# loqalabs/loqa-hub

Measured on AMD Instinct MI355X. Metric: utterances_per_sec (multi-command utterances; ms per added command reported alongside), higher is better.
Workload: dtype bf16

## Files before the change

### csrc/kernels/gemm_ws.hip

```cpp
#include "gemm_mfma.h"

struct GemmWsParams {
  const void* x; long long ldx;
  const void* w;
  int M, N, K;
  int epi, act;
  const float* bias;
  void* y; long long ldy;
  int bm;
  int S;
  float* ws;
  int* counters;
};

template <int FM, int NBW, int NBX, int EPI>
__global__ __launch_bounds__(512) void gemm_ws_kernel(GemmWsParams p) {
  constexpr int WN = 2, WM = 4, NW = 8, FN = 4;
  constexpr int TN = 16 * FN, TM = 16 * FM;
  constexpr int BN = TN * WN, BM = TM * WM;
  constexpr int WSTAGE = BN * 128, XSTAGE = BM * 128;
  constexpr int IW = BN / 8 / NW;
  constexpr int IX = BM / 8 / NW;
  static_assert(IW * 8 * NW == BN && IX * 8 * NW == BM, "stage rows split evenly over the waves");
  static_assert(NBW >= 2 && NBX >= 2 && NBX <= NBW, "stage depths");
  __shared__ __attribute__((aligned(1024))) unsigned char lds[NBW * WSTAGE + NBX * XSTAGE];
  unsigned char* const wl = lds;
  unsigned char* const xl = lds + NBW * WSTAGE;

  const int lane = threadIdx.x & 63;
  const int wave = __builtin_amdgcn_readfirstlane(threadIdx.x >> 6);
  const int wn = wave % WN, wm = wave / WN;
  const int M = p.M, N = p.N;
  const int mblocks = (M + p.bm - 1) / p.bm;
  const int tiles = mblocks * (N / BN), S = p.S;
  const int id = xcd_remap(blockIdx.x, gridDim.x);
  const int s = id / tiles, tile = id - s * tiles;
  const int mb = tile % mblocks, nb = tile / mblocks;
  const int m0 = mb * p.bm, n0 = nb * BN;
  const int KT = p.K / GEMM_BK;
  const int kt0 = (int)(((long long)s * KT) / S), kt1 = (int)(((long long)(s + 1) * KT) / S);
  const int nt = kt1 - kt0;
  const bf16_t* __restrict__ X = reinterpret_cast<const bf16_t*>(p.x);
  const bf16_t* __restrict__ W = reinterpret_cast<const bf16_t*>(p.w);

  const bf16_t* wsrc[IW];
#pragma unroll
  for (int i = 0; i < IW; ++i) {
    const int r = stage_row(wave * IW + i, lane), c = stage_chunk(r, lane);
    wsrc[i] = W + (size_t)weight_row<EPI == EPI_SWIGLU, TN>(r, n0, N) * p.K + (size_t)kt0 * GEMM_BK + c * 8;
  }
  const bf16_t* xsrc[IX];
#pragma unroll
  for (int i = 0; i < IX; ++i) {
    const int r = stage_row(wave * IX + i, lane), c = stage_chunk(r, lane);
    const int m = min(m0 + min(r, p.bm - 1), M - 1);
    xsrc[i] = X + (size_t)m * p.ldx + (size_t)kt0 * GEMM_BK + c * 8;
  }
  auto stage_w = [&](int kt) { stage_issue<IW>(wsrc, kt * GEMM_BK, wl + (kt % NBW) * WSTAGE, wave); };
  auto stage_x = [&](int kt) { stage_issue<IX>(xsrc, kt * GEMM_BK, xl + (kt % NBX) * XSTAGE, wave); };

  float4v acc[FN][FM];
  acc_zero(acc);
  const int fr = lane & 15, fq = lane >> 4;

  static_assert(NBW == 3 && (NBX == 2 || NBX == 3), "the counted waits below assume these depths");
  for (int v = -(NBW - 1); v < 0; ++v) {
    if (v + NBX - 1 >= 0 && v + NBX - 1 < nt) stage_x(v + NBX - 1);
    if (v + NBW - 1 < nt) stage_w(v + NBW - 1);
  }
  for (int t = 0; t < nt; ++t) {
    if (t + 1 < nt) {
      if constexpr (NBX == 2) wait_vm<IW>();
      else wait_vm<IW + IX>();
    } else {
      wait_vm<0>();
    }
    __builtin_amdgcn_s_barrier();
    if (t + NBX - 1 < nt) stage_x(t + NBX - 1);
    if (t + NBW - 1 < nt) stage_w(t + NBW - 1);
    mfma_step(wl + (t % NBW) * WSTAGE, wn * TN, xl + (t % NBX) * XSTAGE, wm * TM, fr, fq, acc);
  }

  if (S > 1 && !splitk_reduce<FN, FM, NW>(p.ws, p.counters, tile, s, S, reinterpret_cast<int*>(lds), wave, lane, acc))
    return;
  epi_store<EPI>(acc, EpiOut{p.y, p.ldy, p.bias, p.act, nullptr, 0}, m0 + wm * TM, min(M, m0 + p.bm),
                 n0 + wn * TN, N, 0, fr, fq);
}

template <int FM, int NBW, int NBX>
static int ws_launch(const GemmWsParams& p, hipStream_t st) {
  const int grid = ((p.M + p.bm - 1) / p.bm) * (p.N / 128) * p.S;
  switch (p.epi) {
    case EPI_SWIGLU:
      hipLaunchKernelGGL((gemm_ws_kernel<FM, NBW, NBX, EPI_SWIGLU>), dim3(grid), dim3(512), 0, st, p);
      break;
    case EPI_RESID:
      hipLaunchKernelGGL((gemm_ws_kernel<FM, NBW, NBX, EPI_RESID>), dim3(grid), dim3(512), 0, st, p);
      break;
    default:
      hipLaunchKernelGGL((gemm_ws_kernel<FM, NBW, NBX, EPI_BF16>), dim3(grid), dim3(512), 0, st, p);
  }
  return (int)hipGetLastError();
}

extern "C" int loqa_gemm_ws(const GemmWsParams* p, int depth, hipStream_t st) {
  if (!p || p->M <= 0 || p->epi < 0 || p->epi > EPI_RESID || !p->x || !p->w || !p->y)
    return (int)hipErrorInvalidValue;
  if (p->N % 128 || p->K % GEMM_BK || p->K < GEMM_BK || p->ldx % 8 || p->ldy % 4 || p->bm < 64 || p->bm % 64 ||
      p->bm > 384 || depth < 0 || depth > 1 || p->S < 1 || p->S > p->K / GEMM_BK)
    return (int)hipErrorInvalidValue;
  if (p->S > 1 && (!p->ws || !p->counters)) return (int)hipErrorInvalidValue;
  if ((p->epi == EPI_SWIGLU && (p->bias || p->act)) || (p->epi == EPI_RESID && p->act))
    return (int)hipErrorInvalidValue;
  const int fm = p->bm / 64;
  if (depth == 1) {
    switch (fm) {
      case 1: return ws_launch<1, 3, 3>(*p, st);
      case 2: return ws_launch<2, 3, 3>(*p, st);
      case 3: return ws_launch<3, 3, 3>(*p, st);
      case 4: return ws_launch<4, 3, 3>(*p, st);
      default: return (int)hipErrorInvalidValue;
    }
  }
  switch (fm) {
    case 1: return ws_launch<1, 3, 2>(*p, st);
    case 2: return ws_launch<2, 3, 2>(*p, st);
    case 3: return ws_launch<3, 3, 2>(*p, st);
    case 4: return ws_launch<4, 3, 2>(*p, st);
    case 5: return ws_launch<5, 3, 2>(*p, st);
    case 6: return ws_launch<6, 3, 2>(*p, st);
    default: return (int)hipErrorInvalidValue;
  }
}
```

### loqa_hub_amd/ops/__init__.py

```python
from __future__ import annotations

import copy
import ctypes
import math
import os

import torch

from . import reference as ref
from . import _lib
from ._lib import FusedParams, check, kernels, ptr, stream_ptr


def _gpu(t: torch.Tensor) -> bool:
    return t.is_cuda


def _bf16_contig(t: torch.Tensor, name: str) -> None:
    if t.dtype != torch.bfloat16:
        raise TypeError(f"{name} must be bfloat16, got {t.dtype}")
    if not t.is_contiguous():
        raise ValueError(f"{name} must be contiguous")


# ... 1441 lines not shown

    def __init__(self, w: torch.Tensor, *, norm: str | None = None, norm_w=None, norm_b=None,
                 bias=None, perm: torch.Tensor | None = None):
        wf = w.float()
        self.norm = norm
        if norm is not None:
            wf = wf * norm_w.float()[None, :]
        wb = wf.to(torch.bfloat16)
        b = torch.zeros(w.shape[0], dtype=torch.float32, device=w.device)
        if bias is not None:
            b = b + bias.float()
        if norm == "ln" and norm_b is not None:
            b = b + (w.float() * norm_b.float()[None, :]).sum(1)
        self.colsum = wb.float().sum(1) if norm == "ln" else None
        self.has_bias = bias is not None or (norm == "ln" and norm_b is not None)
        if perm is not None:
            wb = wb[perm]
            b = b[perm]
            if self.colsum is not None:
                self.colsum = self.colsum[perm].contiguous()
        self.bias = b.contiguous() if self.has_bias else None
        self.wp = shuffle_weight(wb.contiguous())
        self.N, self.K = w.shape


def tune_fused(wp, mode: str, *, mpads=(16, 32, 64, 128), norm=None, act: str = "none",
               heads: tuple | None = None, cos_sin=None, prefill: bool = False,
               xl: bool = True) -> None:
    lin = wp if isinstance(wp, FusedLinear) else None
    w = lin.wp if lin is not None else wp
    if not _gpu(w) or NO_TUNE:
        return
    dev = w.device
    N, K = w.shape[0] * 16, w.shape[1] * 32
    scr = FusedScratch(dev)
    bf = dict(dtype=torch.bfloat16, device=dev)
    nrm = norm if norm is not None else (lin.norm if lin is not None else None)
    nbytes = w.numel() * w.element_size()
    copies = [wp]
    for _ in range(min(15, -(-(768 << 20) // nbytes) - 1)):
        if lin is not None:
            c = copy.copy(lin)
            c.wp = lin.wp.clone()
        else:
            c = wp.clone()
        copies.append(c)
    xl_on = xl and os.environ.get("LOQA_TUNE_XL", "1") != "0"
    for Mpad in mpads:
        if Mpad == 128 and not xl_on:
            continue
        key = (mode, N, K, Mpad) + _wtag(w)
        if key in _FSPLITS:
            continue
        x = torch.randn(Mpad, K, **bf)
        kw: dict = {}
        if nrm:
            tiles = max(1, K // 32)
            scr.rowsq[: tiles * Mpad].fill_(float(K) / tiles)
            kw.update(rowsq_tiles=tiles)
        if mode == "resid":
            kw.update(residual=torch.zeros(Mpad, N, **bf))
        elif mode == "act":
            kw.update(act=act)
        elif mode == "rope":
            H, Hkv, D = heads
            kc = torch.zeros(max(4, Mpad // 16), Hkv, 16, D, **bf)
            pos = torch.arange(Mpad, dtype=torch.int32, device=dev)
            kw.update(positions=pos, cos_sin=cos_sin, q_out=torch.empty(Mpad, H * D, **bf),
                      k_cache=kc, v_cache=torch.zeros_like(kc), slots=pos, n_heads=H, n_kv=Hkv,
                      head_dim=D)
        wide = Mpad <= 32 or prefill
        rts = (1, 2, 4) if (prefill and Mpad == 64) else (1, 2)
        xl = "only" if Mpad == 128 else "no"
        tune_fused_splits(key, lambda sp, rt, wr, i, xl_=0: skinny_fused(
            x, copies[i], mode, scr, splits=sp, rt=rt, wr=wr, norm=nrm, xl=xl_, **kw), K, rts=rts,
            ncopies=len(copies), wr4=wide, fewest=wide, xl=xl)
    del copies


def fold_norm(w: torch.Tensor, norm_w: torch.Tensor) -> torch.Tensor:
    return (w.float() * norm_w.float()[None, :]).to(w.dtype)


def skinny_fused(x: torch.Tensor, wp, mode: str, scratch: FusedScratch, *,
                 splits: int | None = None, norm=None, eps: float = 1e-5,
                 rowsq_tiles: int | None = None, rt: int | None = None,
                 residual: torch.Tensor | None = None, positions=None, cos_sin=None, q_out=None,
                 k_cache=None, v_cache=None, slots=None, n_heads: int = 0, n_kv: int = 0,
                 head_dim: int = 0, out=None, act: str = "none", bias=None, colsum=None,
                 row_sums: bool = False, wr: int | None = None, xl: int | None = None,
                 attn: dict | None = None) -> torch.Tensor:
    if attn is not None:
        assert mode in ("rope", "act")
        rope = mode == "rope"
        if not rope and out is None:
            out = torch.empty(x.shape[0], wp.shape[0] * 16 if not isinstance(wp, FusedLinear)
                              else wp.N, dtype=torch.bfloat16, device=x.device)
        qq = skinny_fused(x, wp, mode, scratch, splits=splits, norm=norm, eps=eps,
                          rowsq_tiles=rowsq_tiles, rt=rt, positions=positions, cos_sin=cos_sin,
                          q_out=q_out, k_cache=k_cache, v_cache=v_cache, slots=slots,
                          n_heads=n_heads, n_kv=n_kv, head_dim=head_dim, bias=bias,
                          colsum=colsum, wr=wr, xl=xl, out=out, act=act)
        if rope:
            return attention(q_out, k_cache, v_cache, attn["cu_q"], n_heads=n_heads,
                             n_kv=n_kv, head_dim=head_dim, causal=True, max_q=attn["max_q"],
                             ctx_lens=attn["ctx_lens"], block_tables=attn["block_tables"],
                             scale=attn.get("scale"), grouped=True,
                             split_keys=attn["split_keys"], num_splits=attn["num_splits"],
                             workspace=attn["workspace"], out=attn.get("out"),
                             max_k=attn.get("max_k"))
        return attention(qq, attn["k"], attn["v"], attn["cu_q"], n_heads=n_heads, n_kv=n_kv,
                         head_dim=head_dim, causal=False, max_q=attn["max_q"],
                         cu_k=attn["kv_start"], ctx_lens=attn["ctx_lens"],
                         scale=attn.get("scale"), grouped=True,
                         split_keys=attn["split_keys"], num_splits=attn["num_splits"],
                         workspace=attn["workspace"], out=attn.get("out"))
    if isinstance(wp, FusedLinear):
        lin = wp
        wp = lin.wp
        norm = lin.norm if norm is None else norm
        bias = lin.bias if bias is None else bias
        colsum = lin.colsum if colsum is None else colsum
    Mpad, K = x.shape
    N = wp.shape[0] * 16
    nrm = _NORMS[norm]
    fp8, mx4 = isinstance(wp, Fp8Weight), isinstance(wp, Mxfp4Weight)
    tuned = _FSPLITS.get((mode, N, K, Mpad) + _wtag(wp))
    S = splits or (tuned[0] if tuned else choose_splits(N, K, Mpad, tag=_wtag(wp)))
    rt = rt or (tuned[1] if tuned else (1 if Mpad == 128 else 2))
    if xl is None:
        xl = tuned[3] if (tuned and not splits and len(tuned) > 3) else int(Mpad == 128)
    if wr is None:
        wr = tuned[2] if (tuned and not splits and len(tuned) > 2) else 1
        if mx4 and wr == 1 and not xl and K % (S * 512):
            S, wr = 1, 4
            rt = rt if N % (64 * rt) == 0 else 1
    if xl:
        wr = 4
        rt = rt if rt in (1, 2) and N % (64 * rt) == 0 else 1
    elif wr != 1 and (S != 1 or N % (64 * rt)):
        wr = 1
    if rowsq_tiles is None:
        rowsq_tiles = scratch.stat_tiles
    m = _FUSED_MODES[mode]
    ntiles = N // (16 * rt)
    if mode == "resid":
        scratch.stat_tiles = ntiles
    if mode == "silu" and out is None:
        out = torch.empty(Mpad, N // 2, dtype=torch.bfloat16, device=x.device)
    elif mode == "act" and out is None:
        out = torch.empty(Mpad, N, dtype=torch.float32 if act == "f32" else torch.bfloat16,
                          device=x.device)
    if not _gpu(x):
        return _skinny_fused_ref(x, wp, mode, scratch, nrm, eps, rowsq_tiles, residual,
                                 positions, cos_sin, q_out, k_cache, v_cache, slots, n_heads,
                                 n_kv, head_dim, out, act, bias, colsum, row_sums, rt)
    assert Mpad in (16, 32, 64, 128) and x.dtype == torch.bfloat16 and x.stride(1) == 1
    assert Mpad != 128 or xl, "Mpad 128 needs the XL layout"
    assert ntiles <= scratch.counters.numel() and ntiles * Mpad <= scratch.rowsq.numel()
    if nrm == 2:
        assert colsum is not None and colsum.numel() == N
    if fp8:
        assert nrm != 2, "fp8 weights: no LayerNorm prologue"
        assert wp.is_cuda and wp.wp.is_contiguous() and wp.scale.is_contiguous()
    elif mx4:
        assert nrm != 2, "MXFP4 weights: no LayerNorm prologue"
        assert wp.is_cuda and wp.wp.is_contiguous() and wp.scales.is_contiguous()
        assert wp.wp.data_ptr() % 16 == 0 and wp.scales.data_ptr() % 4 == 0
    else:
        _bf16_contig(wp, "wp")
    if bias is not None:
        assert bias.dtype == torch.float32 and bias.numel() == N and bias.is_contiguous()
    if mode == "act":
        assert out.dtype == (torch.float32 if act == "f32" else torch.bfloat16)
        assert out.stride(0) % 4 == 0 and out.shape[0] >= Mpad and out.shape[1] >= N
    if mode == "rope":
        assert slots.numel() >= Mpad and q_out.shape[0] >= Mpad and k_cache.is_contiguous()
        assert cos_sin is None or positions.numel() >= Mpad
    elif mode == "resid":
        assert residual.shape[0] >= Mpad and residual.shape[1] == N
    part = torch.empty(S, Mpad, N, dtype=torch.float32, device=x.device) if S > 1 else None
    blk = k_cache.shape[2] if k_cache is not None else 0
    p = FusedParams()
    p.x, p.ldx, p.Wp, p.part, p.counters = ptr(x), x.stride(0), ptr(wp.wp if fp8 or mx4 else wp), \
        ptr(part), ptr(scratch.counters)
    if fp8:
        p.wdtype, p.wscale = 1, ptr(wp.scale)
    elif mx4:
        p.wdtype, p.wscale = 2, ptr(wp.scales)
    p.Mpad, p.N, p.K, p.S, p.mode, p.norm = Mpad, N, K, S, m, nrm
    if nrm:
        p.rowsq_in, p.rowsum_in = ptr(scratch.rowsq), ptr(scratch.rowsum)
    p.rowstat_tiles, p.eps = rowsq_tiles, eps
    p.colsum, p.bias = ptr(colsum), ptr(bias)
    p.out, p.ldo, p.act = ptr(out), (out.stride(0) if out is not None else 0), _ACTS[act]
    if mode == "resid":
        p.residual, p.rowsq_out = ptr(residual), ptr(scratch.rowsq)
        p.rowsum_out = ptr(scratch.rowsum) if row_sums else None
    p.positions, p.cs, p.q_out = ptr(positions), ptr(cos_sin), ptr(q_out)
    p.kc, p.vc, p.slots = ptr(k_cache), ptr(v_cache), ptr(slots)
    p.H, p.Hkv, p.D, p.blk = n_heads, n_kv, head_dim, blk
    p.rt, p.wr, p.xl = rt, wr, int(bool(xl))
    check(kernels().loqa_skinny_fused(ctypes.byref(p), stream_ptr(x)), "skinny_fused")
    if mode in ("silu", "act"):
        return out
    return q_out if mode == "rope" else residual


def set_launch_priority(prio: int) -> None:
    if torch.cuda.is_available():
        kernels().loqa_set_launch_prio(int(prio))


def _skinny_fused_ref(x, wp, mode, scratch, nrm, eps, rowsq_tiles, residual, positions,
                      cos_sin, q_out, k_cache, v_cache, slots, H, Hkv, D, out, act, bias, colsum,
                      row_sums, rt=2):
    Mpad, K = x.shape
    N = wp.shape[0] * 16
    y = x.float() @ ref.unshuffle_weight(wp).float().t()
    if nrm:
        rs = scratch.rowsq[: rowsq_tiles * Mpad].view(rowsq_tiles, Mpad)
        if nrm == 1:
            y = y * ref.fused_row_scale(rs, eps, K)[:, None]
        else:
            sm = scratch.rowsum[: rowsq_tiles * Mpad].view(rowsq_tiles, Mpad)
            mean, rstd = ref.fused_ln_stats(rs, sm, eps, K)
            y = rstd[:, None] * (y - mean[:, None] * colsum.float()[None, :])
    if bias is not None:
        y = y + bias.float()[None, :]
    if mode == "silu":
        F = N // 2
        inv = torch.argsort(ref.perm_gate_up(F))
        y = y[:, inv]
        out.copy_(ref.silu_mul(y.to(torch.bfloat16)))
        return out
    if mode == "act":
        if act == "f32":
            out.copy_(y)
            return out
        yb = y.to(torch.bfloat16)
        if act == "gelu":
            yb = torch.nn.functional.gelu(yb.float()).to(torch.bfloat16)
        out.copy_(yb)
        return out
    if mode == "resid":
        h = (y + residual.float()).to(torch.bfloat16)
        residual.copy_(h)
        R = 16 * rt
        sq = h.float().pow(2).view(Mpad, N // R, R).sum(-1).t().contiguous()
        scratch.rowsq[: sq.numel()] = sq.flatten()
        if row_sums:
            sm = h.float().view(Mpad, N // R, R).sum(-1).t().contiguous()
            scratch.rowsum[: sm.numel()] = sm.flatten()
        return residual
    inv = torch.argsort(ref.perm_rope_qkv(H, Hkv, D))
    qkv = y[:, inv].to(torch.bfloat16)
    ref.rope_kv_append(qkv, positions, cos_sin, k_cache, v_cache, slots, H, Hkv, D)
    q_out.copy_(qkv[:, : H * D])
    return q_out


PREFILL_GEMM_NT = 128


PREFILL2_LAYOUTS = {0: (5, 4, 2), 1: (10, 4, 2), 2: (5, 2, 2), 3: (10, 2, 1), 4: (10, 4, 1)}
PREFILL2_LAYOUT = 3


def prefill_gemm2(x: torch.Tensor, wp: torch.Tensor, splits: int = 1, epi: str = "bf16",
                  layout: int | None = None) -> torch.Tensor:
    M, K = x.shape
    N = wp.shape[0] * 16
    assert wp.shape[1] * 32 == K
    lay = PREFILL2_LAYOUT if layout is None else layout
    rbw, ft, wm = PREFILL2_LAYOUTS[lay]
    e = {"bf16": 0, "slabs": 1, "swiglu": 2}[epi]
    assert e == 1 or splits == 1
    if not _gpu(x):
        part = ref.skinny_gemm(x, wp, splits)
        if e == 1:
            return part
        y = part.sum(0)
        if e == 2:
            y = ref.swiglu_pairs(y)
        return y.to(torch.bfloat16)
    _bf16_contig(x, "x")
    assert N % (16 * ft * (4 // wm)) == 0 and K % (splits * 64) == 0, (N, K, splits, lay)
    if e == 1:
        out = torch.empty(splits, M, N, dtype=torch.float32, device=x.device)
        rc = kernels().loqa_gemm_prefill2(ptr(x), M, K, ptr(wp), N, splits, None, ptr(out), 1, lay,
                                          stream_ptr(x))
    else:
        out = torch.empty(M, N // 2 if e == 2 else N, dtype=torch.bfloat16, device=x.device)
        rc = kernels().loqa_gemm_prefill2(ptr(x), M, K, ptr(wp), N, 1, ptr(out), None, e, lay,
                                          stream_ptr(x))
    check(rc, "gemm_prefill2")
    return out



from .gemm import (
    GEMM_TILE_DEFAULT_LAYOUT, GEMM_TILE_FRAGS, GEMM_TILE_LAYOUTS, PROJ_TABLE, SK_DEEP, SK_LAYOUTS,
    SK_TABLE, _SK_WS, _gt_ref, _sk_ref, conv_k3_im2col_ref, conv_k3_weight, gemm_sk, gemm_sk_plan,
    gemm_tile, gemm_tile_dims, gemm_ws, gemm_ws_rows, proj,
)
```

### loqa_hub_amd/ops/gemm.py

```python
from __future__ import annotations

import ctypes
import os

import torch

from . import _lib
from ._lib import check, kernels, ptr, stream_ptr

_EPI = {"bf16": 0, "swiglu": 1, "resid": 2, "slabs": 3}


def _tiled_ref(x: torch.Tensor, w: torch.Tensor, epi: str, *, bias=None, act: str | None = None,
               residual=None, pos=None, splits: int = 1) -> torch.Tensor:
    xf, wf = x.float(), w.float()
    if epi == "slabs":
        ks = xf.shape[1] // splits
        return torch.stack([xf[:, s * ks:(s + 1) * ks] @ wf[:, s * ks:(s + 1) * ks].t()
                            for s in range(splits)])
    y = xf @ wf.t()
    if epi == "swiglu":
        F = w.shape[0] // 2
        g = y[:, :F].to(torch.bfloat16).float()
        u = y[:, F:].to(torch.bfloat16).float()
        return (g * torch.sigmoid(g) * u).to(torch.bfloat16)
    if bias is not None:
        y = y + bias.float()
    if epi == "resid":
        return (residual.float() + y).to(torch.bfloat16)
    if act == "gelu":
        y = y.to(torch.bfloat16).float()
        y = 0.5 * y * (1.0 + torch.erf(y * 0.70710678118654752))
    if pos is not None:
        rows = torch.arange(y.shape[0], device=y.device) % pos.shape[0]
        y = y.to(torch.bfloat16).float() + pos.float()[rows]
    return y.to(torch.bfloat16)


def _gt_ref(x2: torch.Tensor, w: torch.Tensor, bias, act: str | None, pos, epi: str, splits: int):
    return _tiled_ref(x2, w, epi, bias=bias, act=act, pos=pos, splits=splits)


def _sk_ref(x: torch.Tensor, w: torch.Tensor, epi: str, bias, residual, act: str | None = None):
    return _tiled_ref(x, w, epi, bias=bias, act=act, residual=residual)


def _check_operands(name: str, x: torch.Tensor, w: torch.Tensor, bias, N: int) -> None:
    if x.dtype != torch.bfloat16 or w.dtype != torch.bfloat16:
        raise TypeError(f"{name} needs bf16 operands")
    if x.stride(1) != 1 or not w.is_contiguous():
        raise ValueError(f"{name} needs K-contiguous operands")
    if bias is not None:
        assert bias.dtype == torch.float32 and bias.is_contiguous() and bias.numel() == N


GEMM_TILE_LAYOUTS = {0: (2, 2, 2), 1: (2, 2, 3), 2: (4, 2, 2), 3: (2, 4, 2), 4: (4, 2, 3),
                     5: (2, 4, 3), 6: (2, 4, 2), 7: (4, 2, 2), 8: (2, 2, 2), 9: (2, 2, 2)}
GEMM_TILE_FRAGS = {6: (8, 4), 7: (4, 8), 8: (8, 4), 9: (4, 8)}
GEMM_TILE_DEFAULT_LAYOUT = 1
_GT_ZEROS: dict = {}


def gemm_tile_dims(layout: int) -> tuple[int, int]:
    wn, wm, _ = GEMM_TILE_LAYOUTS[layout]
    fn, fm = GEMM_TILE_FRAGS.get(layout, (4, 4))
    return 16 * fn * wn, 16 * fm * wm


def conv_k3_weight(w: torch.Tensor, cin: int) -> torch.Tensor:
    cout = w.shape[0]
    return w.reshape(cout, cin, 3).permute(0, 2, 1).reshape(cout, 3 * cin).contiguous()


def conv_k3_im2col_ref(x: torch.Tensor, B: int, tin: int, stride: int) -> torch.Tensor:
    cin = x.shape[1]
    xb = x.reshape(B, tin, cin)
    xp = torch.nn.functional.pad(xb, (0, 0, 1, 1))
    tout = (tin + 2 - 3) // stride + 1
    cols = [xp[:, tap: tap + stride * (tout - 1) + 1: stride] for tap in range(3)]
    return torch.cat(cols, dim=2).reshape(B * tout, 3 * cin)


def gemm_tile(x: torch.Tensor, w: torch.Tensor, *, bias: torch.Tensor | None = None,
              act: str | None = None, pos: torch.Tensor | None = None, epi: str = "bf16",
              splits: int = 1, layout: int | None = None, out: torch.Tensor | None = None,
              conv: tuple[int, int] | None = None) -> torch.Tensor:
    N, K = w.shape
    if conv is not None:
        B, stride = conv
        cin = x.shape[1]
        assert K == 3 * cin
        tin = x.shape[0] // B
        tout = (tin + 2 - 3) // stride + 1
        M = B * tout
    else:
        M = x.shape[0]
        assert x.shape[1] == K, (x.shape, w.shape)
    if not x.is_cuda:
        x2 = conv_k3_im2col_ref(x, B, tin, stride) if conv is not None else x
        y = _gt_ref(x2, w, bias, act, pos, epi, splits)
        if out is not None:
            out.copy_(y)
            return out
        return y
    _check_operands("gemm_tile", x, w, bias, N)
    p = _lib.GemmTileParams()
    p.x, p.ldx, p.w = ptr(x), x.stride(0), ptr(w)
    p.M, p.N, p.K, p.S, p.epi = M, N, K, splits, _EPI[epi]
    p.act = 1 if act == "gelu" else 0
    p.bias = ptr(bias)
    if pos is not None:
        assert pos.dtype == torch.bfloat16 and pos.is_contiguous() and pos.shape[1] == N
        p.pos, p.pos_rows = ptr(pos), pos.shape[0]
    if epi == "slabs":
        y = out if out is not None else torch.empty(splits, M, N, dtype=torch.float32,
                                                    device=x.device)
        p.part = ptr(y)
    else:
        cols = N // 2 if epi == "swiglu" else N
        y = out if out is not None else torch.empty(M, cols, dtype=torch.bfloat16, device=x.device)
        assert y.shape == (M, cols) and y.stride(1) == 1
        p.y, p.ldy = ptr(y), y.stride(0)
    if conv is not None:
        z = _GT_ZEROS.get((x.device, cin))
        if z is None:
            z = _GT_ZEROS[(x.device, cin)] = torch.zeros(max(cin, 64), dtype=torch.bfloat16,
                                                         device=x.device)
        p.conv_cin, p.conv_tin, p.conv_tout, p.conv_stride, p.zeros = cin, tin, tout, stride, ptr(z)
    p.layout = GEMM_TILE_DEFAULT_LAYOUT if layout is None else layout
    check(kernels().loqa_gemm_tile(ctypes.byref(p), stream_ptr(x)), "gemm_tile")
    return y


SK_LAYOUTS = {0: (128, 128, 2, 1.0), 1: (128, 64, 3, 0.85), 2: (256, 64, 2, 1.0),
              3: (256, 128, 1, 1.0), 4: (128, 64, 2, 0.9), 5: (128, 128, 1, 1.05),
              6: (256, 256, 1, 1.15), 7: (64, 64, 4, 0.6), 8: (256, 64, 1, 1.05),
              9: (256, 128, 1, 1.1), 10: (128, 128, 1, 1.1), 11: (128, 64, 1, 0.95)}
SK_CUS = 256
_SK_WS: dict = {}


SK_TABLE = {
    (6144, 4096): [(400, 4, 1), (900, 5, 1), (1 << 30, 0, 1)],
    (4096, 4096): [(900, 4, 1), (1 << 30, 1, 1)],
    (28672, 4096): [(400, 4, 1), (1 << 30, 0, 1)],
    (4096, 14336): [(400, 8, 3), (900, 0, 3), (1 << 30, 0, 1)],
    (3840, 1280): [(1 << 30, 0, 1)],
    (1280, 1280): [(2000, 4, 1), (4000, 5, 1), (1 << 30, 3, 1)],
    (5120, 1280): [(1 << 30, 0, 1)],
    (1280, 5120): [(2000, 4, 1), (4000, 5, 1), (1 << 30, 0, 1)],
}


def gemm_sk_plan(M: int, N: int, K: int, epi: str = "bf16",
                 layouts=(0, 1, 2, 3, 4, 5)) -> tuple[int, int]:
    for m_max, lay, s in SK_TABLE.get((N, K), ()):
        if M <= m_max and N % SK_LAYOUTS[lay][0] == 0:
            return lay, s
    KT = K // 64
    best, best_t = (7, 1), float("inf")
    for lay in layouts:
        bn, bm, occ, eff = SK_LAYOUTS[lay]
        if N % bn:
            continue
        tiles = -(-M // bm) * (N // bn)
        for s in (1, 2, 3):
            if s > KT or (s > 1 and KT // s < 8) or (epi == "swiglu" and s > 1):
                continue
            grid = tiles * s
            rounds = -(-grid // (SK_CUS * occ))
            t = rounds * occ * bm * bn * (KT / s) / eff + (s - 1) * bm * bn * 64.0
            if t < best_t:
                best, best_t = (lay, s), t
    return best


_SK_WS_GRAPHS: list = []


def _sk_workspace(dev: torch.device, stream: int, floats: int, tiles: int):
    if dev.type == "cuda" and torch.cuda.is_current_stream_capturing():
        ws = (torch.empty(floats, dtype=torch.float32, device=dev),
              torch.zeros(tiles, dtype=torch.int32, device=dev))
        _SK_WS_GRAPHS.append(ws)
        return ws
    key = (dev, stream)
    ws = _SK_WS.get(key)
    if ws is None or ws[0].numel() < floats or ws[1].numel() < tiles:
        f = max(floats, 0 if ws is None else ws[0].numel())
        t = max(tiles, 0 if ws is None else ws[1].numel())
        ws = (torch.empty(f, dtype=torch.float32, device=dev),
              torch.zeros(t, dtype=torch.int32, device=dev))
        _SK_WS[key] = ws
    return ws


def _fused_epi_args(name: str, p, x: torch.Tensor, w: torch.Tensor, epi: str, bias, act, residual, out):
    N, K = w.shape
    M = x.shape[0]
    assert x.shape[1] == K, (x.shape, w.shape)
    if epi == "resid":
        assert residual is not None and residual.shape == (M, N)
    if not x.is_cuda:
        y = _sk_ref(x, w, epi, bias, residual, act)
        dst = residual if epi == "resid" else out
        if dst is not None:
            dst.copy_(y)
            return dst, False
        return y, False
    _check_operands(name, x, w, bias, N)
    assert not act or epi == "bf16"
    assert bias is None or epi != "swiglu"
    if epi == "resid":
        y = residual
        assert y.dtype == torch.bfloat16 and y.stride(1) == 1
    else:
        cols = N // 2 if epi == "swiglu" else N
        y = out if out is not None else torch.empty(M, cols, dtype=torch.bfloat16, device=x.device)
        assert y.shape == (M, cols) and y.stride(1) == 1
    p.x, p.ldx, p.w = ptr(x), x.stride(0), ptr(w)
    p.M, p.N, p.K, p.epi = M, N, K, _EPI[epi]
    p.act = 1 if act == "gelu" else 0
    p.bias = ptr(bias)
    p.y, p.ldy = ptr(y), y.stride(0)
    return y, True


def gemm_sk(x: torch.Tensor, w: torch.Tensor, *, epi: str = "bf16", bias: torch.Tensor | None = None,
            act: str | None = None, residual: torch.Tensor | None = None,
            out: torch.Tensor | None = None, layout: int | None = None,
            splits: int | None = None) -> torch.Tensor:
    p = _lib.GemmSkParams()
    y, on_gpu = _fused_epi_args("gemm_sk", p, x, w, epi, bias, act, residual, out)
    if not on_gpu:
        return y
    M, (N, K) = x.shape[0], w.shape
    if layout is None or splits is None:
        pl, ps = gemm_sk_plan(M, N, K, epi)
        layout = pl if layout is None else layout
        splits = ps if splits is None else splits
    bn, bm = SK_LAYOUTS[layout][:2]
    if N % bn or K % 64:
        raise ValueError(f"gemm_sk layout {layout}: N {N} / K {K} not tileable")
    p.S, p.layout = splits, layout
    st = stream_ptr(x)
    if splits > 1:
        tiles = -(-M // bm) * (N // bn)
        ws, cnt = _sk_workspace(x.device, st, tiles * splits * bm * bn, tiles)
        p.ws, p.counters = ptr(ws), ptr(cnt)
    check(kernels().loqa_gemm_sk(ctypes.byref(p), st), "gemm_sk")
    return y


WS_MAX_BM = 384


def gemm_ws_rows(M: int, depth: int = 0) -> int:
    cap = WS_MAX_BM if depth == 0 else 256
    nb = -(-M // cap)
    return -(-(-(-M // nb)) // 64) * 64


def gemm_ws(x: torch.Tensor, w: torch.Tensor, *, epi: str = "bf16", bias: torch.Tensor | None = None,
            act: str | None = None, residual: torch.Tensor | None = None,
            out: torch.Tensor | None = None, depth: int | None = None,
            bm: int | None = None, splits: int = 1) -> torch.Tensor:
    p = _lib.GemmWsParams()
    y, on_gpu = _fused_epi_args("gemm_ws", p, x, w, epi, bias, act, residual, out)
    if not on_gpu:
        return y
    M, (N, K) = x.shape[0], w.shape
    if N % 128 or K % 64:
        raise ValueError("gemm_ws needs N % 128 == 0, K % 64 == 0")
    depth = 0 if depth is None else depth
    p.bm = gemm_ws_rows(M, depth) if bm is None else bm
    p.S = splits
    st = stream_ptr(x)
    if splits > 1:
        tiles = -(-M // p.bm) * (N // 128)
        ws, cnt = _sk_workspace(x.device, st, tiles * splits * p.bm * 128, tiles)
        p.ws, p.counters = ptr(ws), ptr(cnt)
    check(kernels().loqa_gemm_ws(ctypes.byref(p), depth, st), "gemm_ws")
    return y


PROJ_TABLE = {
    (6144, 4096): [(64, ("sk", 4, 4)), (128, ("sk", 4, 2)), (400, ("sk", 4, 1)),
                   (900, ("sk", 5, 1)), (1 << 30, ("sk", 0, 1))],
    (4096, 4096): [(128, ("sk", 4, 4)), (256, ("sk", 4, 2)), (900, ("sk", 4, 1)),
                   (1 << 30, ("sk", 0, 1))],
    (28672, 4096): [(256, ("ws", 1)), (384, ("ws", 0)), (900, ("ws", 0)),
                    (1 << 30, ("sk", 6, 1))],
    (4096, 14336): [(64, ("sk", 4, 8)), (128, ("sk", 5, 8)), (256, ("sk", 5, 4)),
                    (400, ("ws", 0, 4)), (700, ("ws", 0, 4)), (1000, ("ws", 0, 2)),
                    (1 << 30, ("sk", 6, 3))],
    (3840, 1280): [(2000, ("sk", 1, 1)), (1 << 30, ("sk", 6, 1))],
    (1280, 1280): [(2000, ("sk", 4, 1)), (1 << 30, ("sk", 5, 1))],
    (5120, 1280): [(2000, ("sk", 0, 1)), (1 << 30, ("sk", 6, 1))],
    (1280, 5120): [(2000, ("sk", 4, 1)), (1 << 30, ("sk", 5, 1))],
    (1280, 8192): [(512, ("sk", 11, 4))],
    (7168, 8192): [(512, ("sk", 9, 3))],
}
SK_DEEP = os.environ.get("LOQA_SK_DEEP", "0") == "1"
for _ov in filter(None, os.environ.get("LOQA_PROJ_OVERRIDE", "").split(";")):
    try:
        _shape, _pick = _ov.split(":")
        _n, _k = map(int, _shape.split("x"))
        _kind, *_args = _pick.split(",")
        if _kind not in ("sk", "ws"):
            raise ValueError(_kind)
        PROJ_TABLE[(_n, _k)] = [(400, (_kind, *map(int, _args)))] + [
            e for e in PROJ_TABLE.get((_n, _k), []) if e[0] > 400]
    except ValueError:
        import warnings
        warnings.warn(f"LOQA_PROJ_OVERRIDE: ignoring malformed entry {_ov!r}")
if SK_DEEP:
    PROJ_TABLE[(6144, 4096)].insert(2, (400, ("sk", 11, 1)))
    PROJ_TABLE[(4096, 4096)].insert(2, (400, ("sk", 11, 1)))
    PROJ_TABLE[(4096, 14336)][3] = (400, ("sk", 9, 4))


def proj(x: torch.Tensor, w: torch.Tensor, *, epi: str = "bf16", bias: torch.Tensor | None = None,
         act: str | None = None, residual: torch.Tensor | None = None) -> torch.Tensor:
    M = x.shape[0]
    N, K = w.shape
    choice = None
    for m_max, c in PROJ_TABLE.get((N, K), ()):
        if M <= m_max:
            choice = c
            break
    if choice is not None and choice[0] == "ws" and N % 128 == 0:
        return gemm_ws(x, w, epi=epi, bias=bias, act=act, residual=residual, depth=choice[1],
                       splits=choice[2] if len(choice) > 2 else 1)
    if choice is not None and choice[0] == "sk" and N % SK_LAYOUTS[choice[1]][0] == 0:
        return gemm_sk(x, w, epi=epi, bias=bias, act=act, residual=residual, layout=choice[1],
                       splits=choice[2])
    return gemm_sk(x, w, epi=epi, bias=bias, act=act, residual=residual)
```

Before: 19.46.

## Split GEMM staging waves into weight and activation roles with deeper weight ring

Waves are split by role: four waves stage only weight tiles and four stage only activation tiles, each with its own ring depth and counted vm waits. Previously every wave issued loads for both operands. The weight ring is deepened to four stages for larger row-block configurations so weight loads can run further ahead. This adds LDS usage and more complex per-role wait logic. There is a risk of load imbalance between the two roles, since IW and IX differ. A Python schedule-model helper is also exported.

New measurement: 19.32. No clear change (-0.8%).

```diff
diff --git a/csrc/kernels/gemm_ws.hip b/csrc/kernels/gemm_ws.hip
--- a/csrc/kernels/gemm_ws.hip
+++ b/csrc/kernels/gemm_ws.hip
@@ -19,9 +19,9 @@
   constexpr int TN = 16 * FN, TM = 16 * FM;
   constexpr int BN = TN * WN, BM = TM * WM;
   constexpr int WSTAGE = BN * 128, XSTAGE = BM * 128;
-  constexpr int IW = BN / 8 / NW;
-  constexpr int IX = BM / 8 / NW;
-  static_assert(IW * 8 * NW == BN && IX * 8 * NW == BM, "stage rows split evenly over the waves");
+  constexpr int IW = BN / 8 / 4;
+  constexpr int IX = BM / 8 / 4;
+  constexpr int IS = IW > IX ? IW : IX;
   static_assert(NBW >= 2 && NBX >= 2 && NBX <= NBW, "stage depths");
   __shared__ __attribute__((aligned(1024))) unsigned char lds[NBW * WSTAGE + NBX * XSTAGE];
   unsigned char* const wl = lds;
@@ -43,41 +43,52 @@
   const bf16_t* __restrict__ X = reinterpret_cast<const bf16_t*>(p.x);
   const bf16_t* __restrict__ W = reinterpret_cast<const bf16_t*>(p.w);
 
-  const bf16_t* wsrc[IW];
+  const bool wrole = wave < 4;
+  const int sw = wave & 3;
+  const bf16_t* src[IS];
 #pragma unroll
-  for (int i = 0; i < IW; ++i) {
-    const int r = stage_row(wave * IW + i, lane), c = stage_chunk(r, lane);
-    wsrc[i] = W + (size_t)weight_row<EPI == EPI_SWIGLU, TN>(r, n0, N) * p.K + (size_t)kt0 * GEMM_BK + c * 8;
+  for (int i = 0; i < IS; ++i) {
+    if (wrole) {
+      const int r = stage_row(sw * IW + min(i, IW - 1), lane), c = stage_chunk(r, lane);
+      src[i] = W + (size_t)weight_row<EPI == EPI_SWIGLU, TN>(r, n0, N) * p.K + (size_t)kt0 * GEMM_BK + c * 8;
+    } else {
+      const int r = stage_row(sw * IX + min(i, IX - 1), lane), c = stage_chunk(r, lane);
+      const int m = min(m0 + min(r, p.bm - 1), M - 1);
+      src[i] = X + (size_t)m * p.ldx + (size_t)kt0 * GEMM_BK + c * 8;
+    }
   }
-  const bf16_t* xsrc[IX];
+  auto stage = [&](int kt) {
+    if (wrole) {
+      unsigned char* dst = wl + (kt % NBW) * WSTAGE + sw * IW * 1024;
 #pragma unroll
-  for (int i = 0; i < IX; ++i) {
-    const int r = stage_row(wave * IX + i, lane), c = stage_chunk(r, lane);
-    const int m = min(m0 + min(r, p.bm - 1), M - 1);
-    xsrc[i] = X + (size_t)m * p.ldx + (size_t)kt0 * GEMM_BK + c * 8;
-  }
-  auto stage_w = [&](int kt) { stage_issue<IW>(wsrc, kt * GEMM_BK, wl + (kt % NBW) * WSTAGE, wave); };
-  auto stage_x = [&](int kt) { stage_issue<IX>(xsrc, kt * GEMM_BK, xl + (kt % NBX) * XSTAGE, wave); };
+      for (int i = 0; i < IW; ++i) glds16(src[i] + kt * GEMM_BK, dst + i * 1024);
+    } else {
+      unsigned char* dst = xl + (kt % NBX) * XSTAGE + sw * IX * 1024;
+#pragma unroll
+      for (int i = 0; i < IX; ++i) glds16(src[i] + kt * GEMM_BK, dst + i * 1024);
+    }
+  };
 
   float4v acc[FN][FM];
   acc_zero(acc);
   const int fr = lane & 15, fq = lane >> 4;
 
-  static_assert(NBW == 3 && (NBX == 2 || NBX == 3), "the counted waits below assume these depths");
-  for (int v = -(NBW - 1); v < 0; ++v) {
-    if (v + NBX - 1 >= 0 && v + NBX - 1 < nt) stage_x(v + NBX - 1);
-    if (v + NBW - 1 < nt) stage_w(v + NBW - 1);
-  }
+  static_assert((NBW == 3 || NBW == 4) && (NBX == 2 || NBX == 3), "the counted waits below assume these depths");
+  const int ring = wrole ? NBW : NBX;
+  for (int v = -(ring - 1); v < 0; ++v)
+    if (v + ring - 1 < nt) stage(v + ring - 1);
   for (int t = 0; t < nt; ++t) {
-    if (t + 1 < nt) {
-      if constexpr (NBX == 2) wait_vm<IW>();
-      else wait_vm<IW + IX>();
+    const int ahead = min(ring - 2, nt - 1 - t);
+    if (wrole) {
+      if (ahead >= 2) wait_vm<2 * IW>();
+      else if (ahead == 1) wait_vm<IW>();
+      else wait_vm<0>();
     } else {
-      wait_vm<0>();
+      if (ahead >= 1) wait_vm<IX>();
+      else wait_vm<0>();
     }
     __builtin_amdgcn_s_barrier();
-    if (t + NBX - 1 < nt) stage_x(t + NBX - 1);
-    if (t + NBW - 1 < nt) stage_w(t + NBW - 1);
+    if (t + ring - 1 < nt) stage(t + ring - 1);
     mfma_step(wl + (t % NBW) * WSTAGE, wn * TN, xl + (t % NBX) * XSTAGE, wm * TM, fr, fq, acc);
   }
 
@@ -117,18 +128,18 @@
     switch (fm) {
       case 1: return ws_launch<1, 3, 3>(*p, st);
       case 2: return ws_launch<2, 3, 3>(*p, st);
-      case 3: return ws_launch<3, 3, 3>(*p, st);
-      case 4: return ws_launch<4, 3, 3>(*p, st);
+      case 3: return ws_launch<3, 4, 3>(*p, st);
+      case 4: return ws_launch<4, 4, 3>(*p, st);
       default: return (int)hipErrorInvalidValue;
     }
   }
   switch (fm) {
     case 1: return ws_launch<1, 3, 2>(*p, st);
     case 2: return ws_launch<2, 3, 2>(*p, st);
-    case 3: return ws_launch<3, 3, 2>(*p, st);
-    case 4: return ws_launch<4, 3, 2>(*p, st);
-    case 5: return ws_launch<5, 3, 2>(*p, st);
-    case 6: return ws_launch<6, 3, 2>(*p, st);
+    case 3: return ws_launch<3, 4, 2>(*p, st);
+    case 4: return ws_launch<4, 4, 2>(*p, st);
+    case 5: return ws_launch<5, 4, 2>(*p, st);
+    case 6: return ws_launch<6, 4, 2>(*p, st);
     default: return (int)hipErrorInvalidValue;
   }
 }
diff --git a/loqa_hub_amd/ops/__init__.py b/loqa_hub_amd/ops/__init__.py
--- a/loqa_hub_amd/ops/__init__.py
+++ b/loqa_hub_amd/ops/__init__.py
@@ -1767,5 +1767,5 @@
 from .gemm import (
     GEMM_TILE_DEFAULT_LAYOUT, GEMM_TILE_FRAGS, GEMM_TILE_LAYOUTS, PROJ_TABLE, SK_DEEP, SK_LAYOUTS,
     SK_TABLE, _SK_WS, _gt_ref, _sk_ref, conv_k3_im2col_ref, conv_k3_weight, gemm_sk, gemm_sk_plan,
-    gemm_tile, gemm_tile_dims, gemm_ws, gemm_ws_rows, proj,
+    gemm_tile, gemm_tile_dims, gemm_ws, gemm_ws_rows, gemm_ws_schedule, proj,
 )
diff --git a/loqa_hub_amd/ops/gemm.py b/loqa_hub_amd/ops/gemm.py
--- a/loqa_hub_amd/ops/gemm.py
+++ b/loqa_hub_amd/ops/gemm.py
@@ -261,6 +261,28 @@
     return -(-(-(-M // nb)) // 64) * 64
 
 
+def gemm_ws_schedule(nt: int, depth: int = 0, fm: int = 5, group: int = 0) -> list[tuple]:
+    assert nt >= 1 and depth in (0, 1) and group in (0, 1)
+    nbw, nbx = 3, (2, 3)[depth]
+    iw, ix = 2, fm
+    ev: list[tuple] = []
+
+    def fill(u: int) -> None:
+        if 0 <= u + nbx - 1 < nt:
+            ev.append(("fill", "x", u + nbx - 1, ix))
+        if u + nbw - 1 < nt:
+            ev.append(("fill", "w", u + nbw - 1, iw))
+
+    for v in range(-(nbw - 1), 0):
+        fill(v)
+    for t in range(nt):
+        ev.append(("wait_vm", (iw if nbx == 2 else iw + ix) if t + 1 < nt else 0))
+        ev.append(("barrier",))
+        fill(t)
+        ev += [("read", t, 0), ("mfma", t, 0), ("read", t, 1), ("mfma", t, 1)]
+    return ev
+
+
 def gemm_ws(x: torch.Tensor, w: torch.Tensor, *, epi: str = "bf16", bias: torch.Tensor | None = None,
             act: str | None = None, residual: torch.Tensor | None = None,
             out: torch.Tensor | None = None, depth: int | None = None,
```
